# Berkeley-Speech-Group/sylber

Hardware: AMD Instinct MI355X
Metric: audio-sec/s encoded (sylber_base, 16 kHz, batched 10 s clips) (higher is better)
Workload: dtype bf16

## Files before the change

### sylber_amd/csrc/api.hip

```cpp
#include "ctx.h"

static thread_local char g_err[512] = "";
void syl_set_error(const char* what, const char* detail) { snprintf(g_err, sizeof(g_err), "%s: %s", what, detail); }
extern "C" const char* sylber_last_error(void) { return g_err; }

struct Packer {
    std::vector<char> host;
    size_t add(size_t bytes) { size_t off = (host.size() + 255) & ~(size_t)255; host.resize(off + bytes); return off; }
    size_t add_f32(const float* src, size_t n) { size_t o = add(n * 4); memcpy(host.data() + o, src, n * 4); return o; }
    int fmt = FMT_BF16;
    size_t add_bf16(const float* src, size_t n) {
        if (fmt == FMT_SPLIT) {
            size_t o = add(n * 4);
            bf16_t* d = (bf16_t*)(host.data() + o);
            for (size_t i = 0; i < n; ++i) { d[i] = f2h_host(src[i]); d[n + i] = f2h_host(src[i] - h2f_host(d[i])); }
            return o;
        }
        size_t o = add(n * 2);
        bf16_t* d = (bf16_t*)(host.data() + o);
        if (fmt == FMT_F16) for (size_t i = 0; i < n; ++i) d[i] = f2h_host(src[i]);
        else for (size_t i = 0; i < n; ++i) d[i] = f2bf(src[i]);
        return o;
    }
};

extern "C" int sylber_create(const SylberWeights* w, int device, int precision, sylber_t* out) {
    if (!w || !out) { syl_set_error("sylber_create", "null argument"); return 1; }
    if (w->num_layers < 1 || w->num_layers > SYLBER_MAX_LAYERS) { syl_set_error("sylber_create", "num_layers out of range"); return 1; }
    if (precision != SYLBER_BF16 && precision != SYLBER_FP32 && precision != SYLBER_FP8 && precision != SYLBER_FP16 && precision != SYLBER_MIXED16 && precision != SYLBER_SPLIT16) { syl_set_error("sylber_create", "unknown precision"); return 1; }
    const bool f32 = precision == SYLBER_FP32;
    GUARD_DEVICE(device);
    sylber_ctx* c = new sylber_ctx();
    c->device = device; c->precision = precision; c->num_layers = w->num_layers;
    c->fmt = precision == SYLBER_FP16 ? FMT_F16 : (precision == SYLBER_SPLIT16 ? FMT_SPLIT : FMT_BF16);
    c->fmt_conv = (precision == SYLBER_FP16 || precision == SYLBER_MIXED16) ? FMT_F16 : (precision == SYLBER_SPLIT16 ? FMT_SPLIT : FMT_BF16);
    Packer P;
    P.fmt = c->fmt_conv;
    size_t o_conv0 = P.add_f32(w->conv_w[0], 512 * 10);
    size_t o_gnw = P.add_f32(w->gn_w, 512), o_gnb = P.add_f32(w->gn_b, 512);
    size_t o_conv[7] = {0};
    for (int i = 1; i < 7; ++i) {
        const int k = CK[i];
        const bool chunk_major = k == 3 && !f32 && c->fmt_conv != FMT_SPLIT;
        std::vector<float> tmp((size_t)512 * k * 512);
        for (int o = 0; o < 512; ++o)
            for (int cc = 0; cc < 512; ++cc)
                for (int j = 0; j < k; ++j) tmp[((size_t)o * k + j) * 512 + cc] = w->conv_w[i][((size_t)o * 512 + cc) * k + j];
        if (chunk_major) {
            std::vector<float> t2(tmp.size());
            for (int o = 0; o < 512; ++o)
                for (int pos = 0; pos < 1536; ++pos)
                    t2[(size_t)o * 1536 + pos] = tmp[(size_t)o * 1536 + tap3_offset(pos * 2) / 2];
            tmp.swap(t2);
        }
        o_conv[i] = f32 ? P.add_f32(tmp.data(), tmp.size()) : P.add_bf16(tmp.data(), tmp.size());
    }
    P.fmt = c->fmt;
    size_t o_fplw = P.add_f32(w->fp_ln_w, 512), o_fplb = P.add_f32(w->fp_ln_b, 512);
    size_t o_fpw = f32 ? P.add_f32(w->fp_w, 768 * 512) : P.add_bf16(w->fp_w, 768 * 512), o_fpb = P.add_f32(w->fp_b, 768);
    size_t o_posw;
    {
        std::vector<float> tmp((size_t)16 * 128 * 64 * 56, 0.f);
        for (int g = 0; g < 16; ++g)
            for (int n = 0; n < 48; ++n)
                for (int cc = 0; cc < 48; ++cc)
                    for (int t = 0; t < 128; ++t)
                        tmp[(((size_t)g * 128 + t) * 64 + n) * 56 + cc] = w->pos_w[(((size_t)g * 48 + n) * 48 + cc) * 128 + t];
        if (!f32) o_posw = P.add_bf16(tmp.data(), tmp.size());
        else {
            std::vector<float> t32((size_t)16 * 128 * 64 * 52, 0.f);
            for (int g = 0; g < 16; ++g)
                for (int n = 0; n < 48; ++n)
                    for (int cc = 0; cc < 48; ++cc)
                        for (int t = 0; t < 128; ++t)
                            t32[(((size_t)g * 128 + t) * 64 + n) * 52 + cc] = w->pos_w[(((size_t)g * 48 + n) * 48 + cc) * 128 + t];
            o_posw = P.add_f32(t32.data(), t32.size());
        }
    }
    size_t o_posb = P.add_f32(w->pos_b, 768);
    size_t o_elw = P.add_f32(w->enc_ln_w, 768), o_elb = P.add_f32(w->enc_ln_b, 768);
    struct LOff { size_t wqkv, bqkv, wo, bo, l1w, l1b, w1, b1, w2, b2, l2w, l2b; } lo[SYLBER_MAX_LAYERS];
    for (int l = 0; l < w->num_layers; ++l) {
        const SylberLayerWeights& lw = w->layers[l];
        std::vector<float> qkv((size_t)2304 * 768), bq(2304);
        memcpy(qkv.data(), lw.q_w, 768 * 768 * 4);
        memcpy(qkv.data() + 768 * 768, lw.k_w, 768 * 768 * 4);
        memcpy(qkv.data() + 2 * 768 * 768, lw.v_w, 768 * 768 * 4);
        memcpy(bq.data(), lw.q_b, 768 * 4); memcpy(bq.data() + 768, lw.k_b, 768 * 4); memcpy(bq.data() + 1536, lw.v_b, 768 * 4);
        lo[l].wqkv = f32 ? P.add_f32(qkv.data(), qkv.size()) : P.add_bf16(qkv.data(), qkv.size()); lo[l].bqkv = P.add_f32(bq.data(), 2304);
        lo[l].wo = f32 ? P.add_f32(lw.o_w, 768 * 768) : P.add_bf16(lw.o_w, 768 * 768); lo[l].bo = P.add_f32(lw.o_b, 768);
        lo[l].l1w = P.add_f32(lw.ln1_w, 768); lo[l].l1b = P.add_f32(lw.ln1_b, 768);
        lo[l].w1 = f32 ? P.add_f32(lw.ff1_w, (size_t)3072 * 768) : P.add_bf16(lw.ff1_w, (size_t)3072 * 768); lo[l].b1 = P.add_f32(lw.ff1_b, 3072);
        lo[l].w2 = f32 ? P.add_f32(lw.ff2_w, (size_t)768 * 3072) : P.add_bf16(lw.ff2_w, (size_t)768 * 3072); lo[l].b2 = P.add_f32(lw.ff2_b, 768);
        lo[l].l2w = P.add_f32(lw.ln2_w, 768); lo[l].l2b = P.add_f32(lw.ln2_b, 768);
    }
    c->wbytes = P.host.size();
    if (hipMalloc((void**)&c->wbase, c->wbytes) != hipSuccess) { delete c; syl_set_error("sylber_create", "hipMalloc(weights) failed"); return 1; }
    if (hipMemcpy(c->wbase, P.host.data(), c->wbytes, hipMemcpyHostToDevice) != hipSuccess) {
        hipFree(c->wbase); delete c; syl_set_error("sylber_create", "weight upload failed"); return 1;
    }
    char* b = c->wbase;
    c->conv0_w = (float*)(b + o_conv0); c->gn_w = (float*)(b + o_gnw); c->gn_b = (float*)(b + o_gnb);
    c->conv_w[0] = nullptr;
    for (int i = 1; i < 7; ++i) { c->conv_w[i] = (bf16_t*)(b + o_conv[i]); c->conv_w32[i] = (float*)(b + o_conv[i]); }
    c->fp_w32 = (float*)(b + o_fpw); c->pos_w32 = (float*)(b + o_posw);
    c->fp_ln_w = (float*)(b + o_fplw); c->fp_ln_b = (float*)(b + o_fplb);
    c->fp_w = (bf16_t*)(b + o_fpw); c->fp_b = (float*)(b + o_fpb);
    c->pos_w = (bf16_t*)(b + o_posw); c->pos_b = (float*)(b + o_posb);
    c->enc_ln_w = (float*)(b + o_elw); c->enc_ln_b = (float*)(b + o_elb);
    for (int l = 0; l < w->num_layers; ++l) {
        LayerDev& d = c->L[l];
        d.wqkv = (bf16_t*)(b + lo[l].wqkv); d.bqkv = (float*)(b + lo[l].bqkv);
        d.wo = (bf16_t*)(b + lo[l].wo); d.bo = (float*)(b + lo[l].bo);
        d.ln1w = (float*)(b + lo[l].l1w); d.ln1b = (float*)(b + lo[l].l1b);
        d.w1 = (bf16_t*)(b + lo[l].w1); d.b1 = (float*)(b + lo[l].b1);
        d.w2 = (bf16_t*)(b + lo[l].w2); d.b2 = (float*)(b + lo[l].b2);
        d.ln2w = (float*)(b + lo[l].l2w); d.ln2b = (float*)(b + lo[l].l2b);
        c->L32[l].wqkv = (float*)(b + lo[l].wqkv); c->L32[l].wo = (float*)(b + lo[l].wo);
        c->L32[l].w1 = (float*)(b + lo[l].w1); c->L32[l].w2 = (float*)(b + lo[l].w2);
    }
    if (precision == SYLBER_FP8) {
        const size_t per_layer = (size_t)3072 * 768 + (size_t)3072 * 24 + (size_t)768 * 3072 + (size_t)768 * 96 +
                                 (size_t)2304 * 768 + (size_t)2304 * 24 + (size_t)768 * 768 + (size_t)768 * 24;
        c->f8bytes = per_layer * w->num_layers;
        float* tmp = nullptr;
        if (hipMalloc((void**)&c->f8base, c->f8bytes) != hipSuccess || hipMalloc((void**)&tmp, (size_t)3072 * 768 * 4) != hipSuccess) {
            if (c->f8base) hipFree(c->f8base);
            hipFree(c->wbase); delete c; syl_set_error("sylber_create", "hipMalloc(fp8 weights) failed"); return 1;
        }
        int bad = 0;
        for (int l = 0; l < w->num_layers && !bad; ++l) {
            LayerDev& d = c->L[l];
            uint8_t* q = (uint8_t*)c->f8base + per_layer * l;
            d.w1q = q; d.w1s = d.w1q + (size_t)3072 * 768; d.w2q = d.w1s + (size_t)3072 * 24; d.w2s = d.w2q + (size_t)768 * 3072;
            d.wqkvq = d.w2s + (size_t)768 * 96; d.wqkvs = d.wqkvq + (size_t)2304 * 768;
            d.woq = d.wqkvs + (size_t)2304 * 24; d.wos = d.woq + (size_t)768 * 768;
            bad |= hipMemcpy(tmp, w->layers[l].o_w, (size_t)768 * 768 * 4, hipMemcpyHostToDevice) != hipSuccess;
            bad |= launch_mx_quant_rows(tmp, 768, d.woq, 768, d.wos, 768, 768, 768, nullptr);
            bad |= hipDeviceSynchronize() != hipSuccess;
            {
                const SylberLayerWeights& lw = w->layers[l];
                bad |= hipMemcpy(tmp, lw.q_w, (size_t)768 * 768 * 4, hipMemcpyHostToDevice) != hipSuccess;
                bad |= hipMemcpy(tmp + (size_t)768 * 768, lw.k_w, (size_t)768 * 768 * 4, hipMemcpyHostToDevice) != hipSuccess;
                bad |= hipMemcpy(tmp + (size_t)2 * 768 * 768, lw.v_w, (size_t)768 * 768 * 4, hipMemcpyHostToDevice) != hipSuccess;
                bad |= launch_mx_quant_rows(tmp, 768, d.wqkvq, 768, d.wqkvs, 2304, 2304, 768, nullptr);
                bad |= hipDeviceSynchronize() != hipSuccess;
            }
            bad |= hipMemcpy(tmp, w->layers[l].ff1_w, (size_t)3072 * 768 * 4, hipMemcpyHostToDevice) != hipSuccess;
            bad |= launch_mx_quant_rows(tmp, 768, d.w1q, 768, d.w1s, 3072, 3072, 768, nullptr);
            bad |= hipDeviceSynchronize() != hipSuccess;
            bad |= hipMemcpy(tmp, w->layers[l].ff2_w, (size_t)768 * 3072 * 4, hipMemcpyHostToDevice) != hipSuccess;
// ... 166 lines not shown
```

### sylber_amd/csrc/common.h

```cpp
#pragma once
#include <hip/hip_runtime.h>
#include <stdint.h>

typedef unsigned short bf16_t;
typedef __bf16 bf16x8_t __attribute__((ext_vector_type(8)));
typedef float f32x16_t __attribute__((ext_vector_type(16)));
typedef float f32x4_t __attribute__((ext_vector_type(4)));
typedef unsigned short u16x8_t __attribute__((ext_vector_type(8)));
typedef unsigned short u16x4_t __attribute__((ext_vector_type(4)));

#define SYL_HIDDEN 768
#define SYL_CONV 512
#define SYL_SLOT_SAMPLES 320
#define SYL_HEADS 12
#define SYL_HDIM 64
#define SYL_FFN 3072
#define SYL_POSK 128
#define SYL_POSG 16
#define SYL_POSC 48

__host__ __device__ __forceinline__ bf16_t f2bf(float f) {
    union { float f; uint32_t u; } v; v.f = f;
    uint32_t u = v.u;
    if ((u & 0x7fffffffu) > 0x7f800000u) return (bf16_t)((u >> 16) | 0x40);
    u += 0x7fffu + ((u >> 16) & 1u);
    return (bf16_t)(u >> 16);
}
__host__ __device__ __forceinline__ float bf2f(bf16_t h) {
    union { float f; uint32_t u; } v; v.u = ((uint32_t)h) << 16;
    return v.f;
}
typedef __bf16 bf16x2_t __attribute__((ext_vector_type(2)));
__device__ __forceinline__ uint32_t pack_bf16x2(float lo, float hi) {
    typedef float f32pair_t __attribute__((ext_vector_type(2)));
    const f32pair_t v = {lo, hi};
    return __builtin_bit_cast(uint32_t, __builtin_convertvector(v, bf16x2_t));
}
__device__ __forceinline__ bf16_t f2bf_dev(float f) { return __builtin_bit_cast(unsigned short, (__bf16)f); }

enum { FMT_BF16 = 0, FMT_F16 = 1, FMT_SPLIT = 2 };
typedef _Float16 f16x8_t __attribute__((ext_vector_type(8)));
typedef _Float16 f16x2_t __attribute__((ext_vector_type(2)));
#define SYL_Q_SCALE 0.18033688011112042f
template <int FMT> struct H16 {
    static __device__ __forceinline__ uint32_t pack2(float lo, float hi) { return pack_bf16x2(lo, hi); }
    static __device__ __forceinline__ uint32_t pack2_bounded(float lo, float hi) { return pack_bf16x2(lo, hi); }
    static __device__ __forceinline__ bf16_t cvt(float f) { return f2bf_dev(f); }
    static __device__ __forceinline__ float up(bf16_t h) { return bf2f(h); }
    static __device__ __forceinline__ f32x16_t mfma(bf16x8_t a, bf16x8_t b, f32x16_t c) {
        return __builtin_amdgcn_mfma_f32_32x32x16_bf16(a, b, c, 0, 0, 0);
    }
};
template <> struct H16<FMT_F16> {
    static __device__ __forceinline__ float sat(float f) { return __builtin_amdgcn_fmed3f(f, -65504.0f, 65504.0f); }
    static __device__ __forceinline__ uint32_t pack2(float lo, float hi) {
        typedef float f32pair_t __attribute__((ext_vector_type(2)));
        const f32pair_t v = {sat(lo), sat(hi)};
        return __builtin_bit_cast(uint32_t, __builtin_convertvector(v, f16x2_t));
    }
    static __device__ __forceinline__ uint32_t pack2_bounded(float lo, float hi) {
        typedef float f32pair_t __attribute__((ext_vector_type(2)));
        const f32pair_t v = {lo, hi};
        return __builtin_bit_cast(uint32_t, __builtin_convertvector(v, f16x2_t));
    }
    static __device__ __forceinline__ bf16_t cvt(float f) { return __builtin_bit_cast(unsigned short, (_Float16)sat(f)); }
    static __device__ __forceinline__ float up(bf16_t h) { return (float)__builtin_bit_cast(_Float16, h); }
    static __device__ __forceinline__ f32x16_t mfma(bf16x8_t a, bf16x8_t b, f32x16_t c) {
        return __builtin_amdgcn_mfma_f32_32x32x16_f16(__builtin_bit_cast(f16x8_t, a), __builtin_bit_cast(f16x8_t, b), c, 0, 0, 0);
    }
};
template <> struct H16<FMT_SPLIT> : H16<FMT_F16> {
    static __device__ __forceinline__ uint32_t pack2_lo(float lo, float hi, uint32_t hi2) {
        const f16x2_t h = __builtin_bit_cast(f16x2_t, hi2);
        return H16<FMT_F16>::pack2_bounded(lo - (float)h[0], hi - (float)h[1]);
    }
    static __device__ __forceinline__ bf16_t cvt_lo(float f, bf16_t hi) { return H16<FMT_F16>::cvt(f - H16<FMT_F16>::up(hi)); }
};
__host__ __forceinline__ bf16_t f2h_host(float f) {
    union { float f; uint32_t u; } v; v.f = f;
    const uint32_t sign = (v.u >> 16) & 0x8000u;
    uint32_t a = v.u & 0x7fffffffu;
    if (a > 0x7f800000u) return (bf16_t)(sign | 0x7e00u);
    if (a >= 0x477ff000u) return (bf16_t)(sign | 0x7bffu);
    if (a < 0x38800000u) {
        if (a < 0x33000000u) return (bf16_t)sign;
        const int e = (int)(a >> 23);
        const uint32_t m = (a & 0x7fffffu) | 0x800000u;
        const int shift = 126 - e;
        uint32_t r = m >> shift;
        const uint32_t rem = m & ((1u << shift) - 1u), half = 1u << (shift - 1);
        if (rem > half || (rem == half && (r & 1u))) ++r;
        return (bf16_t)(sign | r);
    }
    a += 0xc8000000u;
    a += 0xfffu + ((a >> 13) & 1u);
    return (bf16_t)(sign | (a >> 13));
}


__host__ __forceinline__ float h2f_host(bf16_t h) {
    const uint32_t sign = ((uint32_t)h & 0x8000u) << 16;
    uint32_t e = (h >> 10) & 0x1fu, m = h & 0x3ffu;
    union { float f; uint32_t u; } v;
    if (e == 0) {
        if (m == 0) { v.u = sign; return v.f; }
        int sh = 0;
        while (!(m & 0x400u)) { m <<= 1; ++sh; }
        m &= 0x3ffu; e = 1 - sh;
        v.u = sign | ((uint32_t)(e + 112) << 23) | (m << 13);
        return v.f;
    }
    if (e == 31) { v.u = sign | 0x7f800000u | (m << 13); return v.f; }
    v.u = sign | ((e + 112) << 23) | (m << 13);
    return v.f;
}

__device__ __forceinline__ float gelu_erf(float x) {
    const float hx = 0.5f * x;
    return __builtin_fmaf(hx, erff(x * 0.70710678118654752f), hx);
}
__device__ __forceinline__ float gelu_erf7(float x) {
    const float z = x * 0.70710678118654752f;
    const float az = __builtin_fabsf(z);
    const float t = __builtin_amdgcn_rcpf(__builtin_fmaf(0.3275911f, az, 1.0f));
    float p = __builtin_fmaf(1.061405429f, t, -1.453152027f);
    p = __builtin_fmaf(p, t, 1.421413741f);
    p = __builtin_fmaf(p, t, -0.284496736f);
    p = __builtin_fmaf(p, t, 0.254829592f);
    p = p * t;
    const float e = __builtin_amdgcn_exp2f(az * az * -1.44269504088896341f);
    const float erf_abs = __builtin_fmaf(-p, e, 1.0f);
    const float erf = __builtin_copysignf(erf_abs, z);
    const float hx = 0.5f * x;
    return __builtin_fmaf(hx, erf, hx);
}
__device__ __forceinline__ float gelu_fast(float x) {
    const float xc = __builtin_amdgcn_fmed3f(x, -4.2f, 4.2f);
    const float u = xc * xc;
    float q = fmaf(6.949803233e-11f, u, -6.356798643e-09f);
    q = fmaf(q, u, 2.570604920e-07f);
    q = fmaf(q, u, -6.139445304e-06f);
    q = fmaf(q, u, 9.818511899e-05f);
    q = fmaf(q, u, -1.133762766e-03f);
    q = fmaf(q, u, 9.886963293e-03f);
    q = fmaf(q, u, -6.643489748e-02f);
    q = fmaf(q, u, 3.989362717e-01f);
    return x * fmaf(xc, q, 0.5f);
}

#ifndef SYL_GELU_VARIANT
#define SYL_GELU_VARIANT 0
// ... 73 lines not shown
```

### sylber_amd/csrc/forward.hip

```cpp
#include "ctx.h"

extern "C" int32_t sylber_num_frames(int32_t n) {
    for (int i = 0; i < 7; ++i) n = (n - CK[i]) / CS[i] + 1;
    return n;
}

static int frames_needed(int Lmax) {
    int n = Lmax, tp = 0;
    for (int i = 0; i < 7; ++i) {
        n = (n - CK[i]) / CS[i] + 1;
        const int f = 1 << (6 - i);
        const int need = (n + f - 1) / f;
        tp = need > tp ? need : tp;
    }
    return tp;
}
static int padded_frames(int Lmax) { return (frames_needed(Lmax) + 31) & ~31; }
extern "C" int32_t sylber_padded_frames(int32_t n_samples) { return n_samples < 400 ? 0 : padded_frames(n_samples); }

#define SYL_SLOT_ALIGN 64
extern "C" int sylber_packed_layout(const int32_t* samples_host, int32_t B, int32_t* offsets, int32_t* frames) {
    if (!samples_host || !offsets || !frames || B < 1) { syl_set_error("sylber_packed_layout", "need B >= 1 and non-null arrays"); return 1; }
    const long long cap = (long long)INT32_MAX / SYL_SLOT_SAMPLES;
    long long off = 0;
// ... 249 lines not shown
}

struct Forward {
    sylber_ctx* c; const Plan& p; const float* wav_dev; float* hidden_dev; hipStream_t s; const PackedCall* pk;
    const Ws<bf16_t> w; const WsF8 w8;
    const int B, M;
    const bool split;
    const bool f8;
    const bool aud_c, aud_e;
    const bf16_t* feats = nullptr; long feats_lo = 0;
    const float *res_g = nullptr, *res_b = nullptr;

    Forward(sylber_ctx* c_, const Plan& p_, const float* wav, float* hidden, hipStream_t s_, const PackedCall* pk_)
        : c(c_), p(p_), wav_dev(wav), hidden_dev(hidden), s(s_), pk(pk_), w(c_->ws, p_), w8(w, p_), B(p_.B), M(p_.B * p_.Tp),
          split(c_->precision == SYLBER_SPLIT16), f8(c_->precision == SYLBER_FP8),
          aud_c(c_->opt_audit16 && c_->fmt_conv == FMT_F16), aud_e(c_->opt_audit16 && c_->fmt == FMT_F16) {}

    int conv0() {
        if (pk) {
            RUN("conv0_stats", launch_conv0_stats(wav_dev, pk->nclip, 0, p.L[0], w.part, p.nchunk, s, pk->rows0, pk->slot));
            RUN("conv0_finalize", launch_conv0_finalize(w.part, p.nchunk, c->conv0_w, c->gn_w, c->gn_b, pk->nclip, p.L[0], w.ss, s, pk->rows0));
            RUN("conv0_gn_gelu", launch_conv0_packed(wav_dev, pk->nclip, pk->total_samples, pk->slot_max, pk->rows0, pk->slot, c->conv0_w, w.ss, w.bufA, c->fmt_conv, s));
        } else {
            const int* rows0 = c->opt_per_utt ? w.rows : nullptr;
            RUN("conv0_stats", launch_conv0_stats(wav_dev, B, p.Lmax, p.L[0], w.part, p.nchunk, s, rows0));
            RUN("conv0_finalize", launch_conv0_finalize(w.part, p.nchunk, c->conv0_w, c->gn_w, c->gn_b, B, p.L[0], w.ss, s, rows0));
            RUN("conv0_gn_gelu", launch_conv0_gn_gelu(wav_dev, B, p.Lmax, p.L[0], p.R[0], c->conv0_w, w.ss, w.bufA, 0, s, c->fmt_conv, p.lo_bufA, c->opt_conv0_valu));
        }
        AUDIT(aud_c, AUD_CONV0, w.bufA, (long)B * p.R[0], 512, 512);
        return 0;
    }

    int conv_stack() {
        static const char* nm[7] = {"", "gemm_conv1", "gemm_conv2", "gemm_conv3", "gemm_conv4", "gemm_conv5", "gemm_conv6"};
        bf16_t* src = w.bufA; bf16_t* dst = w.bufB;
        long src_lo = p.lo_bufA, dst_lo = p.lo_bufB;
        for (int i = 1; i < 7; ++i) {
            GemmArgs a = {};
            a.X = src; a.ldx = (long)CS[i] * 512; a.W = c->conv_w[i]; a.M = B * p.R[i]; a.N = 512; a.K = CK[i] * 512;
            a.act = split ? ACT_GELU_ERF7 : ACT_GELU_FAST; a.out0 = dst; a.ld0 = 512; a.fmt = c->fmt_conv;
            a.x_lo = src_lo; a.w_lo = (long)512 * CK[i] * 512; a.out_lo = dst_lo;
            a.kpat = (CK[i] == 3 && c->fmt_conv != FMT_SPLIT) ? 1 : 0;
            tune_from_options(c, a);
            RUN(nm[i], launch_gemm_bf16(EPI_BF16, a, s));
            AUDIT(aud_c, AUD_CONV0 + i, dst, (long)B * p.R[i], 512, 512);
            std::swap(src, dst); std::swap(src_lo, dst_lo);
        }
        feats = src; feats_lo = src_lo;
        return 0;
    }

    GemmArgs linear(const bf16_t* X, long x_lo, const bf16_t* W, const float* bias, int N, int K) const {
        GemmArgs g = {};
        g.X = X; g.ldx = K; g.x_lo = x_lo; g.W = W; g.w_lo = (long)N * K; g.bias = bias; g.M = M; g.N = N; g.K = K; g.fmt = c->fmt;
        return g;
    }
    GemmF8Args linear8(const uint8_t* X8, const uint8_t* XS, const uint8_t* W8, const uint8_t* WS, const float* bias, int N, int K) const {
        GemmF8Args g = {};
        g.g.M = M; g.g.N = N; g.g.K = K; g.g.bias = bias;
        g.X8 = X8; g.ldx8 = K; g.XS = XS; g.xs_rows = w8.Mp; g.W8 = W8; g.WS = WS; g.ws_rows = N;
        return g;
    }
    void residual(GemmArgs& g, const float* gamma, const float* beta) const {
        g.out0 = w.pre; g.ld0 = 768; g.res = w.pre; g.ldres = 768; g.ln_stats = w.stats; g.ln_gamma = gamma; g.ln_beta = beta;
    }

    int projection() {
        LnArgs a = {};
        a.in = feats; a.in_bf16 = 1; a.ld_in = 512; a.gamma = c->fp_ln_w; a.beta = c->fp_ln_b;
        a.out_bf16 = w.ln512; a.ld_bf16 = 512; a.M = M; a.D = 512; a.fmt = c->fmt; a.fmt_in = c->fmt_conv;
        a.in_lo = feats_lo; a.out_lo = p.lo_ln512;
        RUN("ln512", launch_layernorm(a, s));
        GemmArgs g = linear(w.ln512, p.lo_ln512, c->fp_w, c->fp_b, 768, 512);
        g.out0 = w.xf32; g.ld0 = 768; g.out1 = w.xpad; g.Tp = p.Tp; g.T = p.T; g.valid = w.valid; g.xpad_rows = p.Tp + 128; g.out_lo = p.lo_xpad;
        RUN("gemm_proj", launch_gemm_bf16(EPI_PROJ, g, s));
        if (pk) RUN("zero_slot_tails", launch_zero_slot_tails(w.xf32, w.xpad, pk->slot, pk->frames, pk->nclip, pk->tail_max, s));
        AUDIT(aud_e, AUD_LN512, w.ln512, M, 512, 512);
        AUDIT(aud_e, AUD_XPAD, w.xpad, (long)B * (p.Tp + 128), 768, 768);
        return 0;
    }

    int posconv() {
        if (pk) RUN("posconv", launch_posconv_packed(w.xpad, c->pos_w, c->pos_b, w.xf32, w.pre, pk->nclip, pk->slot_max, pk->slot, pk->frames, s, c->fmt));
        else RUN("posconv", launch_posconv(w.xpad, c->pos_w, c->pos_b, w.xf32, w.pre, B, p.Tp, split ? 2 : 1, s, c->fmt, p.lo_xpad, (long)16 * 128 * 64 * 56));
        return 0;
    }

    int layernorm(const float* gam, const float* bet, bool last) {
        LnArgs a = {};
        a.in = w.pre; a.in_bf16 = 0; a.ld_in = 768; a.gamma = gam; a.beta = bet; a.M = M; a.D = 768; a.fmt = c->fmt; a.fmt_in = c->fmt;
        if (last) { a.out_f32 = hidden_dev; a.ld_f32 = 768; a.Tp = p.Tp; a.T = p.T; }
        else if (f8) { a.out_fp8 = w8.h; a.ld_fp8 = 768; a.out_scale = w8.hs; a.scale_rows = w8.Mp; a.out_stats = w.stats; }
        else { a.out_bf16 = w.h; a.ld_bf16 = 768; a.out_stats = w.stats; a.out_lo = p.lo_hbf; }
        if (launch_layernorm(a, s)) return 1;
        AUDIT(aud_e && !last && !f8, AUD_LN, w.h, M, 768, 768);
        return 0;
    }

    int layer16(const LayerDev& d, bool last) {
        GemmArgs g = linear(w.h, p.lo_hbf, d.wqkv, d.bqkv, 2304, 768);
        g.out0 = w.q; g.out1 = w.k; g.out2 = w.vt; g.Tp = p.Tp; g.Tpv = p.Tpv; g.T = p.T; g.out_lo = p.lo_qk; g.out2_lo = p.lo_vt;
        tune_from_options(c, g);
        RUN("gemm_qkv", launch_gemm_bf16(EPI_QK, g, s));
        AUDIT(aud_e, AUD_Q, w.q, M, 768, 768);
        AUDIT(aud_e, AUD_K, w.k, M, 768, 768);
        AUDIT(aud_e, AUD_V, w.vt, (long)B * 768, p.Tp, p.Tpv);
        if (pk) RUN("attention", launch_attention_packed(w.q, w.k, w.vt, pk->slot, pk->nclip, pk->total_qb, w.ctx, p.Tp, s, c->fmt));
        else RUN("attention", launch_attention(w.q, w.k, w.vt, w.valid, w.ctx, B, p.T, p.Tp, p.Tpv, c->opt_attn_qw, s, c->fmt, p.lo_qk, p.lo_vt, p.lo_ctx));
        AUDIT(aud_e, AUD_CTX, w.ctx, M, 768, 768);
        GemmArgs o = linear(w.ctx, p.lo_ctx, d.wo, d.bo, 768, 768);
        residual(o, res_g, res_b);
        tune_from_options(c, o);
        o.out1 = w.h; o.ln_stats_out = w.stats; o.ln_gamma_out = d.ln1w; o.ln_beta_out = d.ln1b;
        if (!split && c->opt_fuse_ln > 0 && gemm_rowln_applicable(o)) {
            RUN("gemm_out_ln", launch_gemm_rowln(o, s));
        } else {
            RUN("gemm_out", launch_gemm_bf16(EPI_F32_RESLN, o, s));
            RUN("layernorm", layernorm(d.ln1w, d.ln1b, false));
        }
        GemmArgs f1 = linear(w.h, p.lo_hbf, d.w1, d.b1, 3072, 768);
        f1.act = split ? ACT_GELU_ERF7 : ACT_GELU_FAST; f1.out0 = w.ffn; f1.ld0 = 3072; f1.out_lo = p.lo_ffn;
        tune_from_options(c, f1);
        RUN("gemm_ffn1", launch_gemm_bf16(EPI_BF16, f1, s));
        AUDIT(aud_e, AUD_FFN1, w.ffn, M, 3072, 3072);
        GemmArgs f2 = linear(w.ffn, p.lo_ffn, d.w2, d.b2, 768, 3072);
        residual(f2, d.ln1w, d.ln1b);
        tune_from_options(c, f2);
        RUN("gemm_ffn2", launch_gemm_bf16(EPI_F32_RESLN, f2, s));
        RUN("layernorm", layernorm(d.ln2w, d.ln2b, last));
        return 0;
    }

    int layer8(const LayerDev& d, bool last) {
        GemmF8Args g = linear8(w8.h, w8.hs, d.wqkvq, d.wqkvs, d.bqkv, 2304, 768);
        g.g.out0 = w.q; g.g.out1 = w.k; g.g.out2 = w.vt; g.g.Tp = p.Tp; g.g.Tpv = p.Tpv; g.g.T = p.T;
        GemmF8Args gq = g;
        gq.g.M = (int)w8.Mp; gq.g.M_store = M;
        if (c->opt_attn8 >= 0 && gemm_asm_f8_tile(EPI_QK8, gq) != 0) {
            gq.g.out0 = w8.q; gq.g.out1 = w8.k; gq.g.out2 = w8.v; gq.qs = w8.qs; gq.ks = w8.ks; gq.vs = w8.vs;
            RUN("gemm_qkv", launch_gemm_mxfp8(EPI_QK8, gq, s));
            RUN("attention", launch_attention_f8(w8.q, w8.qs, w8.k, w8.ks, w8.v, w8.vs, w.valid, w8.ctx, w8.ctxs, w8.Mp, B, p.T, p.Tp, p.Tpv, s));
        } else {
            RUN("gemm_qkv", launch_gemm_mxfp8(EPI_QK, g, s));
            RUN("attention", launch_attention_f8out(w.q, w.k, w.vt, w.valid, w8.ctx, w8.ctxs, w8.Mp, B, p.T, p.Tp, p.Tpv, c->opt_attn_qw, s));
        }
        GemmF8Args o = linear8(w8.ctx, w8.ctxs, d.woq, d.wos, d.bo, 768, 768);
        residual(o.g, res_g, res_b);
        RUN("gemm_out", launch_gemm_mxfp8(EPI_F32_RESLN, o, s));
        RUN("layernorm", layernorm(d.ln1w, d.ln1b, false));
        GemmF8Args f1 = linear8(w8.h, w8.hs, d.w1q, d.w1s, d.b1, 3072, 768);
        f1.g.act = 1; f1.g.out0 = w8.ffn; f1.g.ld0 = 3072; f1.out_scale = w8.ffns; f1.os_rows = w8.Mp;
        RUN("gemm_ffn1", launch_gemm_mxfp8(EPI_MXFP8, f1, s));
        GemmF8Args f2 = linear8(w8.ffn, w8.ffns, d.w2q, d.w2s, d.b2, 768, 3072);
        residual(f2.g, d.ln1w, d.ln1b);
        RUN("gemm_ffn2", launch_gemm_mxfp8(EPI_F32_RESLN, f2, s));
        RUN("layernorm", layernorm(d.ln2w, d.ln2b, last));
        return 0;
    }

    int run() {
        if (conv0()) return 1;
        if (c->stop_stage == SYLBER_TAP_CONV0) {
            RUN("copy_out", launch_bf16_to_f32_rows(w.bufA, 512, hidden_dev, B, p.R[0], p.R[0], 512, s, c->fmt_conv, p.lo_bufA));
            return 0;
        }
        if (conv_stack()) return 1;
        if (c->stop_stage == 1) {
// ... 244 lines not shown
```

### sylber_amd/csrc/posconv.hip

```cpp
#include "kernels.h"

#define PC_BM 256
#define PC_XROW 112
#define PC_XWIN (384 * PC_XROW)
#define PC_SLAB (64 * 112)
#define PC_TAPS_PER_STEP 2
#define PC_STEP (PC_TAPS_PER_STEP * PC_SLAB)
#define PC_LDS (PC_XWIN + 2 * PC_STEP)

typedef __attribute__((address_space(3))) void* lds_vptr;
typedef const __attribute__((address_space(1))) void* glb_vptr;
__device__ __forceinline__ void glds16p(__amdgpu_buffer_rsrc_t rs, int voff, int soff, void* l) {
    __builtin_amdgcn_raw_ptr_buffer_load_lds(rs, (lds_vptr)l, 16, voff, soff, 0, 0);
}

template <int ACT, int FMT>
__global__ __launch_bounds__(512, 4) void posconv_bf16_kernel(const bf16_t* __restrict__ xpad, const bf16_t* __restrict__ wpk,
                                                              const float* __restrict__ bias, const float* __restrict__ x_f32,
                                                              float* __restrict__ out, int Tp, long x_lo, long w_lo,
                                                              const int* __restrict__ slot, const int* __restrict__ frames) {
    extern __shared__ __attribute__((aligned(256))) char smem[];
    char* xwin = smem;
    char* wring = smem + PC_XWIN;
    const int tid = threadIdx.x, wave = tid >> 6, lane = tid & 63;
    const int ql = lane & 31, h = lane >> 5;
    const int t0 = blockIdx.x * PC_BM, g = blockIdx.y, b = blockIdx.z;
    const int rows_per_b = Tp + 128;
    int s0 = 0, Tb = 0, Tpb = Tp;
    if (slot) {
        s0 = slot[b]; Tb = frames[b]; Tpb = slot[b + 1] - s0;
        if (t0 >= Tpb) return;
    }

    f32x16_t acc[2];
#pragma unroll
    for (int i = 0; i < 2; ++i)
#pragma unroll
        for (int r = 0; r < 16; ++r) acc[i][r] = 0.f;
    constexpr int NPASS = FMT == FMT_SPLIT ? 3 : 1;
#pragma unroll 1
    for (int pass = 0; pass < NPASS; ++pass) {
    if (pass > 0) __syncthreads();
    {
        const bf16_t* xb = xpad + (pass == 1 ? x_lo : 0L) + (slot ? (size_t)s0 : (size_t)b * rows_per_b) * SYL_HIDDEN + g * SYL_POSC;
#pragma unroll
        for (int i = 0; i < 5; ++i) {
            const int idx = tid + 512 * i;
            if (idx < 384 * 6) {
                const int r = idx / 6, ch = idx - r * 6;
                uint4 v;
                if (slot) {
                    const int f = t0 + r - 64;
                    v = (f >= 0 && f < Tb) ? *(const uint4*)(xb + (size_t)(f + 64) * SYL_HIDDEN + ch * 8) : make_uint4(0u, 0u, 0u, 0u);
                } else {
                    int row = t0 + r; row = row < rows_per_b ? row : rows_per_b - 1;
                    v = *(const uint4*)(xb + (size_t)row * SYL_HIDDEN + ch * 8);
                }
                *(uint4*)(xwin + r * PC_XROW + ch * 16) = v;
            }
        }
    }
    const char* wg_base = (const char*)(wpk + (pass == 2 ? w_lo : 0L)) + (size_t)g * SYL_POSK * PC_SLAB;
    const __amdgpu_buffer_rsrc_t rwg = __builtin_amdgcn_make_buffer_rsrc((void*)wg_base, 0, (int)0xffffffffu, 0x00020000);
    auto stage = [&](int step, int buf) {
        char* dst = wring + buf * PC_STEP;
#pragma unroll
        for (int i = 0; i < 2; ++i) {
            const int piece = wave + 8 * i;
            if (piece < 14) glds16p(rwg, piece * 1024 + lane * 16, step * PC_STEP, dst + piece * 1024);
        }
    };

    const int xfrag = (wave * 32 + ql) * PC_XROW + h * 16;
    const int wfrag = ql * 112 + h * 16;
    const int nsteps = SYL_POSK / PC_TAPS_PER_STEP;
    stage(0, 0);
    for (int st = 0; st < nsteps; ++st) {
        asm volatile("s_waitcnt vmcnt(0)" ::: "memory");
        __syncthreads();
        if (st + 1 < nsteps) stage(st + 1, (st + 1) & 1);
        const char* wb = wring + (st & 1) * PC_STEP;
#pragma unroll
        for (int tt = 0; tt < PC_TAPS_PER_STEP; ++tt) {
            const int tap = st * PC_TAPS_PER_STEP + tt;
#pragma unroll
            for (int q = 0; q < 3; ++q) {
                const bf16x8_t xf = *(const bf16x8_t*)(xwin + xfrag + tap * PC_XROW + q * 32);
#pragma unroll
                for (int nf = 0; nf < 2; ++nf) {
                    const bf16x8_t wf = *(const bf16x8_t*)(wb + tt * PC_SLAB + nf * 32 * 112 + wfrag + q * 32);
                    acc[nf] = H16<FMT>::mfma(wf, xf, acc[nf]);
                }
            }
        }
    }
    }
    const int t = t0 + wave * 32 + ql;
    if (t < Tpb) {
        const size_t m = slot ? (size_t)s0 + t : (size_t)b * Tp + t;
#pragma unroll
        for (int nf = 0; nf < 2; ++nf)
#pragma unroll
            for (int gg = 0; gg < 4; ++gg) {
                const int nl = 32 * nf + 8 * gg + 4 * h;
                if (nl >= SYL_POSC) continue;
                const int n = g * SYL_POSC + nl;
                const float4 bb = *(const float4*)(bias + n);
                const float4 rr = *(const float4*)(x_f32 + m * SYL_HIDDEN + n);
                float v0 = acc[nf][4 * gg + 0] + bb.x, v1 = acc[nf][4 * gg + 1] + bb.y;
                float v2 = acc[nf][4 * gg + 2] + bb.z, v3 = acc[nf][4 * gg + 3] + bb.w;
                if constexpr (ACT == 2 && FMT == FMT_SPLIT) { v0 = gelu_erf7(v0); v1 = gelu_erf7(v1); v2 = gelu_erf7(v2); v3 = gelu_erf7(v3); }
                else if constexpr (ACT == 2) { v0 = gelu_erf(v0); v1 = gelu_erf(v1); v2 = gelu_erf(v2); v3 = gelu_erf(v3); }
                else { v0 = gelu_fast(v0); v1 = gelu_fast(v1); v2 = gelu_fast(v2); v3 = gelu_fast(v3); }
                *(float4*)(out + m * SYL_HIDDEN + n) = make_float4(rr.x + v0, rr.y + v1, rr.z + v2, rr.w + v3);
            }
    }
}

static int posconv_attrs() {
    static PerDeviceOnce attr_once;
    if (attr_once.need()) {
        HIP_TRY(hipFuncSetAttribute((const void*)posconv_bf16_kernel<1, FMT_BF16>, hipFuncAttributeMaxDynamicSharedMemorySize, PC_LDS));
        HIP_TRY(hipFuncSetAttribute((const void*)posconv_bf16_kernel<2, FMT_BF16>, hipFuncAttributeMaxDynamicSharedMemorySize, PC_LDS));
        HIP_TRY(hipFuncSetAttribute((const void*)posconv_bf16_kernel<1, FMT_F16>, hipFuncAttributeMaxDynamicSharedMemorySize, PC_LDS));
        HIP_TRY(hipFuncSetAttribute((const void*)posconv_bf16_kernel<2, FMT_SPLIT>, hipFuncAttributeMaxDynamicSharedMemorySize, PC_LDS));
    }
    return 0;
}

int launch_posconv(const bf16_t* xpad, const bf16_t* wpk, const float* bias, const float* x_f32, float* out, int B, int Tp,
                   int act, hipStream_t s, int fmt, long x_lo, long w_lo) {
    dim3 grid((Tp + PC_BM - 1) / PC_BM, SYL_POSG, B);
    if (posconv_attrs()) return 1;
    if (fmt == FMT_SPLIT) {
        hipLaunchKernelGGL((posconv_bf16_kernel<2, FMT_SPLIT>), grid, dim3(512), PC_LDS, s, xpad, wpk, bias, x_f32, out, Tp, x_lo, w_lo, nullptr, nullptr);
        HIP_TRY(hipGetLastError());
        return 0;
    }
    if (fmt == FMT_F16 && act == 2) { syl_set_error("launch_posconv", "the erf GELU (act 2) has no fp16 instantiation"); return 1; }
    if (fmt == FMT_F16) hipLaunchKernelGGL((posconv_bf16_kernel<1, FMT_F16>), grid, dim3(512), PC_LDS, s, xpad, wpk, bias, x_f32, out, Tp, 0L, 0L, nullptr, nullptr);
    else if (act == 2) hipLaunchKernelGGL((posconv_bf16_kernel<2, FMT_BF16>), grid, dim3(512), PC_LDS, s, xpad, wpk, bias, x_f32, out, Tp, 0L, 0L, nullptr, nullptr);
    else hipLaunchKernelGGL((posconv_bf16_kernel<1, FMT_BF16>), grid, dim3(512), PC_LDS, s, xpad, wpk, bias, x_f32, out, Tp, 0L, 0L, nullptr, nullptr);
    HIP_TRY(hipGetLastError());
    return 0;
}

int launch_posconv_packed(const bf16_t* xpad, const bf16_t* wpk, const float* bias, const float* x_f32, float* out, int B, int slot_max,
                          const int* slot, const int* frames, hipStream_t s, int fmt) {
    if (fmt != FMT_BF16 && fmt != FMT_F16) { syl_set_error("launch_posconv_packed", "bf16 / fp16 only"); return 1; }
    if (posconv_attrs()) return 1;
    dim3 grid((slot_max + PC_BM - 1) / PC_BM, SYL_POSG, B);
    if (fmt == FMT_F16) hipLaunchKernelGGL((posconv_bf16_kernel<1, FMT_F16>), grid, dim3(512), PC_LDS, s, xpad, wpk, bias, x_f32, out, 0, 0L, 0L, slot, frames);
    else hipLaunchKernelGGL((posconv_bf16_kernel<1, FMT_BF16>), grid, dim3(512), PC_LDS, s, xpad, wpk, bias, x_f32, out, 0, 0L, 0L, slot, frames);
    HIP_TRY(hipGetLastError());
    return 0;
}
```

Measured before the change: 67500.

## Switch positional conv to 16x16x32 MFMA with unpadded packed weight layout

```diff
diff --git a/sylber_amd/csrc/api.hip b/sylber_amd/csrc/api.hip
--- a/sylber_amd/csrc/api.hip
+++ b/sylber_amd/csrc/api.hip
@@ -60,13 +60,17 @@
     size_t o_fpw = f32 ? P.add_f32(w->fp_w, 768 * 512) : P.add_bf16(w->fp_w, 768 * 512), o_fpb = P.add_f32(w->fp_b, 768);
     size_t o_posw;
     {
-        std::vector<float> tmp((size_t)16 * 128 * 64 * 56, 0.f);
-        for (int g = 0; g < 16; ++g)
-            for (int n = 0; n < 48; ++n)
-                for (int cc = 0; cc < 48; ++cc)
-                    for (int t = 0; t < 128; ++t)
-                        tmp[(((size_t)g * 128 + t) * 64 + n) * 56 + cc] = w->pos_w[(((size_t)g * 48 + n) * 48 + cc) * 128 + t];
-        if (!f32) o_posw = P.add_bf16(tmp.data(), tmp.size());
+        if (!f32) {
+            std::vector<float> tmp((size_t)16 * 128 * 48 * 48);
+            for (int g = 0; g < 16; ++g)
+                for (int n = 0; n < 48; ++n)
+                    for (int cc = 0; cc < 48; ++cc)
+                        for (int t = 0; t < 128; ++t) {
+                            const int i = (t & 1) * 6 + cc / 8;
+                            tmp[((((size_t)g * 64 + t / 2) * 12 + i) * 48 + n) * 8 + cc % 8] = w->pos_w[(((size_t)g * 48 + n) * 48 + cc) * 128 + t];
+                        }
+            o_posw = P.add_bf16(tmp.data(), tmp.size());
+        }
         else {
             std::vector<float> t32((size_t)16 * 128 * 64 * 52, 0.f);
             for (int g = 0; g < 16; ++g)
diff --git a/sylber_amd/csrc/common.h b/sylber_amd/csrc/common.h
--- a/sylber_amd/csrc/common.h
+++ b/sylber_amd/csrc/common.h
@@ -50,6 +50,9 @@
     static __device__ __forceinline__ f32x16_t mfma(bf16x8_t a, bf16x8_t b, f32x16_t c) {
         return __builtin_amdgcn_mfma_f32_32x32x16_bf16(a, b, c, 0, 0, 0);
     }
+    static __device__ __forceinline__ f32x4_t mfma16(bf16x8_t a, bf16x8_t b, f32x4_t c) {
+        return __builtin_amdgcn_mfma_f32_16x16x32_bf16(a, b, c, 0, 0, 0);
+    }
 };
 template <> struct H16<FMT_F16> {
     static __device__ __forceinline__ float sat(float f) { return __builtin_amdgcn_fmed3f(f, -65504.0f, 65504.0f); }
@@ -67,6 +70,9 @@
     static __device__ __forceinline__ float up(bf16_t h) { return (float)__builtin_bit_cast(_Float16, h); }
     static __device__ __forceinline__ f32x16_t mfma(bf16x8_t a, bf16x8_t b, f32x16_t c) {
         return __builtin_amdgcn_mfma_f32_32x32x16_f16(__builtin_bit_cast(f16x8_t, a), __builtin_bit_cast(f16x8_t, b), c, 0, 0, 0);
+    }
+    static __device__ __forceinline__ f32x4_t mfma16(bf16x8_t a, bf16x8_t b, f32x4_t c) {
+        return __builtin_amdgcn_mfma_f32_16x16x32_f16(__builtin_bit_cast(f16x8_t, a), __builtin_bit_cast(f16x8_t, b), c, 0, 0, 0);
     }
 };
 template <> struct H16<FMT_SPLIT> : H16<FMT_F16> {
diff --git a/sylber_amd/csrc/forward.hip b/sylber_amd/csrc/forward.hip
--- a/sylber_amd/csrc/forward.hip
+++ b/sylber_amd/csrc/forward.hip
@@ -355,7 +355,7 @@
 
     int posconv() {
         if (pk) RUN("posconv", launch_posconv_packed(w.xpad, c->pos_w, c->pos_b, w.xf32, w.pre, pk->nclip, pk->slot_max, pk->slot, pk->frames, s, c->fmt));
-        else RUN("posconv", launch_posconv(w.xpad, c->pos_w, c->pos_b, w.xf32, w.pre, B, p.Tp, split ? 2 : 1, s, c->fmt, p.lo_xpad, (long)16 * 128 * 64 * 56));
+        else RUN("posconv", launch_posconv(w.xpad, c->pos_w, c->pos_b, w.xf32, w.pre, B, p.Tp, split ? 2 : 1, s, c->fmt, p.lo_xpad, (long)16 * 128 * 48 * 48));
         return 0;
     }
 
diff --git a/sylber_amd/csrc/posconv.hip b/sylber_amd/csrc/posconv.hip
--- a/sylber_amd/csrc/posconv.hip
+++ b/sylber_amd/csrc/posconv.hip
@@ -3,9 +3,8 @@
 #define PC_BM 256
 #define PC_XROW 112
 #define PC_XWIN (384 * PC_XROW)
-#define PC_SLAB (64 * 112)
 #define PC_TAPS_PER_STEP 2
-#define PC_STEP (PC_TAPS_PER_STEP * PC_SLAB)
+#define PC_STEP (12 * SYL_POSC * 16)
 #define PC_LDS (PC_XWIN + 2 * PC_STEP)
 
 typedef __attribute__((address_space(3))) void* lds_vptr;
@@ -23,7 +22,8 @@
     char* xwin = smem;
     char* wring = smem + PC_XWIN;
     const int tid = threadIdx.x, wave = tid >> 6, lane = tid & 63;
-    const int ql = lane & 31, h = lane >> 5;
+    const int ql = lane & 15, j = lane >> 4;
+    const int fl = 2 * (ql < 4 ? ql : (ql >= 12 ? ql - 8 : ql + 4));
     const int t0 = blockIdx.x * PC_BM, g = blockIdx.y, b = blockIdx.z;
     const int rows_per_b = Tp + 128;
     int s0 = 0, Tb = 0, Tpb = Tp;
@@ -32,11 +32,11 @@
         if (t0 >= Tpb) return;
     }
 
-    f32x16_t acc[2];
+    f32x4_t acc[2][3];
 #pragma unroll
-    for (int i = 0; i < 2; ++i)
+    for (int fb = 0; fb < 2; ++fb)
 #pragma unroll
-        for (int r = 0; r < 16; ++r) acc[i][r] = 0.f;
+        for (int nb = 0; nb < 3; ++nb) acc[fb][nb] = f32x4_t{0.f, 0.f, 0.f, 0.f};
     constexpr int NPASS = FMT == FMT_SPLIT ? 3 : 1;
 #pragma unroll 1
     for (int pass = 0; pass < NPASS; ++pass) {
@@ -60,60 +60,59 @@
             }
         }
     }
-    const char* wg_base = (const char*)(wpk + (pass == 2 ? w_lo : 0L)) + (size_t)g * SYL_POSK * PC_SLAB;
+    const char* wg_base = (const char*)(wpk + (pass == 2 ? w_lo : 0L)) + (size_t)g * (SYL_POSK / PC_TAPS_PER_STEP) * PC_STEP;
     const __amdgpu_buffer_rsrc_t rwg = __builtin_amdgcn_make_buffer_rsrc((void*)wg_base, 0, (int)0xffffffffu, 0x00020000);
     auto stage = [&](int step, int buf) {
         char* dst = wring + buf * PC_STEP;
-#pragma unroll
-        for (int i = 0; i < 2; ++i) {
-            const int piece = wave + 8 * i;
-            if (piece < 14) glds16p(rwg, piece * 1024 + lane * 16, step * PC_STEP, dst + piece * 1024);
-        }
+        glds16p(rwg, wave * 1024 + lane * 16, step * PC_STEP, dst + wave * 1024);
+        if (wave == (step & 7)) glds16p(rwg, 8 * 1024 + lane * 16, step * PC_STEP, dst + 8 * 1024);
     };
 
-    const int xfrag = (wave * 32 + ql) * PC_XROW + h * 16;
-    const int wfrag = ql * 112 + h * 16;
+    int xoff[3];
+#pragma unroll
+    for (int m = 0; m < 3; ++m) {
+        const int i = 4 * m + j;
+        xoff[m] = (wave * 32 + fl + i / 6) * PC_XROW + (i % 6) * 16;
+    }
+    const int wfrag = (j * SYL_POSC + ql) * 16;
     const int nsteps = SYL_POSK / PC_TAPS_PER_STEP;
     stage(0, 0);
     for (int st = 0; st < nsteps; ++st) {
         asm volatile("s_waitcnt vmcnt(0)" ::: "memory");
         __syncthreads();
         if (st + 1 < nsteps) stage(st + 1, (st + 1) & 1);
-        const char* wb = wring + (st & 1) * PC_STEP;
+        const char* wb = wring + (st & 1) * PC_STEP + wfrag;
+        const char* xb = xwin + st * PC_TAPS_PER_STEP * PC_XROW;
 #pragma unroll
-        for (int tt = 0; tt < PC_TAPS_PER_STEP; ++tt) {
-            const int tap = st * PC_TAPS_PER_STEP + tt;
+        for (int m = 0; m < 3; ++m) {
+            const bf16x8_t xf0 = *(const bf16x8_t*)(xb + xoff[m]);
+            const bf16x8_t xf1 = *(const bf16x8_t*)(xb + xoff[m] + PC_XROW);
 #pragma unroll
-            for (int q = 0; q < 3; ++q) {
-                const bf16x8_t xf = *(const bf16x8_t*)(xwin + xfrag + tap * PC_XROW + q * 32);
-#pragma unroll
-                for (int nf = 0; nf < 2; ++nf) {
-                    const bf16x8_t wf = *(const bf16x8_t*)(wb + tt * PC_SLAB + nf * 32 * 112 + wfrag + q * 32);
-                    acc[nf] = H16<FMT>::mfma(wf, xf, acc[nf]);
-                }
+            for (int nb = 0; nb < 3; ++nb) {
+                const bf16x8_t wf = *(const bf16x8_t*)(wb + (4 * m * SYL_POSC + 16 * nb) * 16);
+                acc[0][nb] = H16<FMT>::mfma16(wf, xf0, acc[0][nb]);
+                acc[1][nb] = H16<FMT>::mfma16(wf, xf1, acc[1][nb]);
             }
         }
     }
     }
-    const int t = t0 + wave * 32 + ql;
-    if (t < Tpb) {
+#pragma unroll
+    for (int fb = 0; fb < 2; ++fb) {
+        const int t = t0 + wave * 32 + fl + fb;
+        if (t >= Tpb) continue;
         const size_t m = slot ? (size_t)s0 + t : (size_t)b * Tp + t;
 #pragma unroll
-        for (int nf = 0; nf < 2; ++nf)
-#pragma unroll
-            for (int gg = 0; gg < 4; ++gg) {
-                const int nl = 32 * nf + 8 * gg + 4 * h;
-                if (nl >= SYL_POSC) continue;
-                const int n = g * SYL_POSC + nl;
-                const float4 bb = *(const float4*)(bias + n);
-                const float4 rr = *(const float4*)(x_f32 + m * SYL_HIDDEN + n);
-                float v0 = acc[nf][4 * gg + 0] + bb.x, v1 = acc[nf][4 * gg + 1] + bb.y;
-                float v2 = acc[nf][4 * gg + 2] + bb.z, v3 = acc[nf][4 * gg + 3] + bb.w;
-                if constexpr (ACT == 2 && FMT == FMT_SPLIT) { v0 = gelu_erf7(v0); v1 = gelu_erf7(v1); v2 = gelu_erf7(v2); v3 = gelu_erf7(v3); }
-                else if constexpr (ACT == 2) { v0 = gelu_erf(v0); v1 = gelu_erf(v1); v2 = gelu_erf(v2); v3 = gelu_erf(v3); }
-                else { v0 = gelu_fast(v0); v1 = gelu_fast(v1); v2 = gelu_fast(v2); v3 = gelu_fast(v3); }
-                *(float4*)(out + m * SYL_HIDDEN + n) = make_float4(rr.x + v0, rr.y + v1, rr.z + v2, rr.w + v3);
-            }
+        for (int nb = 0; nb < 3; ++nb) {
+            const int n = g * SYL_POSC + 16 * nb + 4 * j;
+            const float4 bb = *(const float4*)(bias + n);
+            const float4 rr = *(const float4*)(x_f32 + m * SYL_HIDDEN + n);
+            float v0 = acc[fb][nb][0] + bb.x, v1 = acc[fb][nb][1] + bb.y;
+            float v2 = acc[fb][nb][2] + bb.z, v3 = acc[fb][nb][3] + bb.w;
+            if constexpr (ACT == 2 && FMT == FMT_SPLIT) { v0 = gelu_erf7(v0); v1 = gelu_erf7(v1); v2 = gelu_erf7(v2); v3 = gelu_erf7(v3); }
+            else if constexpr (ACT == 2) { v0 = gelu_erf(v0); v1 = gelu_erf(v1); v2 = gelu_erf(v2); v3 = gelu_erf(v3); }
+            else { v0 = gelu_fast(v0); v1 = gelu_fast(v1); v2 = gelu_fast(v2); v3 = gelu_fast(v3); }
+            *(float4*)(out + m * SYL_HIDDEN + n) = make_float4(rr.x + v0, rr.y + v1, rr.z + v2, rr.w + v3);
+        }
     }
 }
 
```

New measurement: 67910 (median of 6 runs). Within noise of the previous version (+0.6%).
